# pyannote/pyannote-audio

Hardware: AMD Instinct MI355X
Metric: audio-hours/sec (real-time factor) for speaker-diarization-3.1 pipeline (higher is better)
Workload: dtype f32

## Files before the change

### pyannote-audio_amd/csrc/common.h

```cpp
#pragma once
#include <hip/hip_runtime.h>
#include <stdint.h>
#include <stdio.h>

typedef float f32x4 __attribute__((ext_vector_type(4)));
typedef float f32x16 __attribute__((ext_vector_type(16)));
typedef unsigned int u32x4 __attribute__((ext_vector_type(4)));

#define MFMA16(a, b, c) __builtin_amdgcn_mfma_f32_16x16x4f32((a), (b), (c), 0, 0, 0)
#define MFMA32(a, b, c) __builtin_amdgcn_mfma_f32_32x32x2f32((a), (b), (c), 0, 0, 0)

#define PA_INTERNAL __attribute__((visibility("hidden")))
PA_INTERNAL int pa_mfcc_frontend(const float* wav, long wav_len, long chunk_stride, int B, int N, int T, int hop,
                                 int center, int log_mels, const float* window, const float* fft_tw,
                                 const float* mel_w, const int* mel_lo, const int* mel_hi, int nmel,
                                 const float* dct, int n_mfcc, float* mel_buf, unsigned int* chunk_max, float* out,
                                 int rows, void* stream);
PA_INTERNAL int pa_stats_pool_rows_any(const float* feat, int B, int T0, int Tp, int C, int ld, const float* masks,
                                       int S, int Fm, const int* nearest_idx, float* stats, int ld_stats,
                                       const float* aff_scale, const float* aff_shift, void* stream);
PA_INTERNAL void pa_square_from_condensed(const double* cond, int n, long ld, double* S, void* stream);
PA_INTERNAL void pa_row_norms_f64(const double* X, int N, int D, double* nrm, void* stream);

#include "workspace.h"
namespace pa {

inline long square_ld(int n) { return ((long)n + 7) & ~7L; }
PA_INTERNAL bool square_fits(int n);

struct LfState {
  double *S, *mind0;
  int *nb0, *g_size, *g_cid;
  unsigned long long* mail;
  int* status;
};
PA_INTERNAL bool lf_wanted(int n);
PA_INTERNAL void lf_layout(Carver& c, int n, LfState& s);
PA_INTERNAL int lf_launch(const double* cond, int n, double* Z, const LfState& s, long long* stats, hipStream_t st);

void set_error(const char* fmt, ...);

hipError_t fill_async(void* dst, int value, size_t nbytes, hipStream_t st);

int* tile_counters();
}
#include "tile_queue.h"
namespace pa {

struct ProfScope {
  ProfScope(const char* name, void* stream, double flops, double bytes);
  ~ProfScope();
  long idx_;
  void* stream_;
};

#define PA_CHECK_LAUNCH(name)                                              \
  do {                                                                     \
    hipError_t e__ = hipGetLastError();                                    \
    if (e__ != hipSuccess) {                                               \
      pa::set_error("%s: launch failed: %s", name, hipGetErrorString(e__)); \
      return e__ == hipErrorOutOfMemory ? 2 : 1;                           \
    }                                                                      \
  } while (0)

#define PA_REQUIRE(cond, ...)        \
  do {                               \
    if (!(cond)) {                   \
      pa::set_error(__VA_ARGS__);    \
      return 3;                      \
    }                                \
  } while (0)

__device__ __forceinline__ float wave_sum(float v) {
#pragma unroll
  for (int o = 32; o > 0; o >>= 1) v += __shfl_xor(v, o, 64);
  return v;
}
__device__ __forceinline__ double wave_sum_d(double v) {
#pragma unroll
  for (int o = 32; o > 0; o >>= 1) v += __shfl_xor(v, o, 64);
  return v;
}

struct MinPair {
  double d;
  int i;
};
__device__ __forceinline__ MinPair min_pair(MinPair a, MinPair b) {
  if (b.i >= 0 && (a.i < 0 || b.d < a.d || (b.d == a.d && b.i < a.i))) return b;
  return a;
}

template <int NW>
__device__ __forceinline__ float block_sum(float v, float* red) {
  v = wave_sum(v);
  const int lane = threadIdx.x & 63, w = threadIdx.x >> 6;
  __syncthreads();
  if (lane == 0) red[w] = v;
  __syncthreads();
  float s = 0.f;
#pragma unroll
  for (int i = 0; i < NW; ++i) s += red[i];
  return s;
}

__device__ __forceinline__ float leaky_relu(float x) { return x > 0.f ? x : 0.01f * x; }
__device__ __forceinline__ float gelu_erf(float x) { return 0.5f * x * (1.f + erff(x * 0.70710678118654752440f)); }

static inline int cdiv(long a, long b) { return (int)((a + b - 1) / b); }

}
```

### pyannote-audio_amd/csrc/emb_fbank.hip

```cpp
#include "common.h"

namespace pa {

constexpr int FB_WIN = 400, FB_SHIFT = 160, FB_NFFT = 512, FB_HALF = 256, FB_NBIN = 257;
constexpr int FB_FPB = 4;

struct cplx {
  float x, y;
};
__device__ __forceinline__ cplx cmul(cplx a, cplx b) {
  return {a.x * b.x - a.y * b.y, a.x * b.y + a.y * b.x};
}

template <bool kRagged>
__global__ __launch_bounds__(256) void k_fbank(const float* __restrict__ wav, long wav_len,
                                               long chunk_stride, int T, float scale, float preemph,
                                               const float* __restrict__ window,
                                               const float2* __restrict__ tw256,
                                               const float2* __restrict__ tw512,
                                               const float* __restrict__ mel_w,
                                               const int* __restrict__ mel_lo,
                                               const int* __restrict__ mel_hi, int nmel, float eps,
                                               float* __restrict__ out, const int64_t* __restrict__ offs,
                                               const int* __restrict__ lens) {
  __shared__ float2 bufA[FB_FPB][FB_HALF];
  __shared__ float2 bufB[FB_FPB][FB_HALF];
  __shared__ float2 s_tw256[FB_HALF];
  __shared__ float xs[FB_FPB][FB_NFFT + 1];
  const int tid = threadIdx.x, lane = tid & 63, wv = tid >> 6;
  const int b = blockIdx.y;
  const int t = blockIdx.x * FB_FPB + wv;
  int Tb = T;
  long base = (long)b * chunk_stride + (long)t * FB_SHIFT;
  if constexpr (kRagged) {
    const int n = lens[b];
    Tb = n < FB_WIN ? 0 : 1 + (n - FB_WIN) / FB_SHIFT;
    if ((int)blockIdx.x * FB_FPB >= Tb) return;
    base = offs[b] + (long)t * FB_SHIFT;
  }
  for (int i = tid; i < FB_HALF; i += 256) s_tw256[i] = tw256[i];
  const bool active = t < Tb;
  float2 w512[5];
#pragma unroll
  for (int i = 0; i < 5; ++i) w512[i] = lane + 64 * i <= FB_HALF ? tw512[lane + 64 * i] : make_float2(0.f, 0.f);

  float x[7];
  float s = 0.f;
#pragma unroll
  for (int i = 0; i < 7; ++i) {
    const int j = lane + 64 * i;
    float v = 0.f;
    if (active && j < FB_WIN) {
      const long g = base + j;
      v = (g < wav_len ? wav[g] : 0.f) * scale;
    }
    x[i] = v;
    s += v;
  }
  const float mean = wave_sum(s) / (float)FB_WIN;
  float* xw = xs[wv];
#pragma unroll
  for (int i = 0; i < 7; ++i) {
    const int j = lane + 64 * i;
    if (j < FB_WIN) xw[j + 1] = x[i] - mean;
  }
  if (lane == 0) xw[0] = x[0] - mean;
  __syncthreads();
  float y[8];
#pragma unroll
  for (int i = 0; i < 8; ++i) {
    const int j = lane + 64 * i;
    float v = 0.f;
    if (j < FB_WIN) v = (xw[j + 1] - preemph * xw[j]) * window[j];
    y[i] = v;
  }
  __syncthreads();
#pragma unroll
  for (int i = 0; i < 8; ++i) xw[lane + 64 * i] = y[i];
  __syncthreads();
  float2* A = bufA[wv];
  float2* Bf = bufB[wv];
#pragma unroll
  for (int i = 0; i < 4; ++i) {
    const int n = lane + 64 * i;
    A[n] = make_float2(xw[2 * n], xw[2 * n + 1]);
  }
  __syncthreads();

  float2* src = A;
  float2* dst = Bf;
#pragma unroll
  for (int pass = 0; pass < 4; ++pass) {
    const int Ns = 1 << (2 * pass);
    const int j = lane;
    const int k = j & (Ns - 1);
    const int tstep = 64 >> (2 * pass);
    cplx v[4];
#pragma unroll
    for (int r = 0; r < 4; ++r) {
      const float2 d = src[j + 64 * r];
      const float2 w = s_tw256[(r * k * tstep) & 255];
      v[r] = cmul({d.x, d.y}, {w.x, w.y});
    }
    const cplx t0 = {v[0].x + v[2].x, v[0].y + v[2].y};
    const cplx t1 = {v[0].x - v[2].x, v[0].y - v[2].y};
    const cplx t2 = {v[1].x + v[3].x, v[1].y + v[3].y};
    const cplx d13 = {v[1].x - v[3].x, v[1].y - v[3].y};
    const cplx t3 = {d13.y, -d13.x};
    const int j0 = ((j - k) << 2) + k;
    dst[j0] = make_float2(t0.x + t2.x, t0.y + t2.y);
    dst[j0 + Ns] = make_float2(t1.x + t3.x, t1.y + t3.y);
    dst[j0 + 2 * Ns] = make_float2(t0.x - t2.x, t0.y - t2.y);
    dst[j0 + 3 * Ns] = make_float2(t1.x - t3.x, t1.y - t3.y);
    __syncthreads();
    float2* tmp = src;
    src = dst;
    dst = tmp;
  }
#pragma unroll
  for (int i = 0; i < 5; ++i) {
    const int k = lane + 64 * i;
    if (k <= FB_HALF) {
      const float2 zk = src[k & 255];
      const float2 zc0 = src[(FB_HALF - k) & 255];
      const cplx zc = {zc0.x, -zc0.y};
      const cplx e = {0.5f * (zk.x + zc.x), 0.5f * (zk.y + zc.y)};
      const cplx dd = {0.5f * (zk.x - zc.x), 0.5f * (zk.y - zc.y)};
      const cplx o = {dd.y, -dd.x};
      const float2 w = w512[i];
      const cplx wo = cmul(o, {w.x, w.y});
      const float re = e.x + wo.x, im = e.y + wo.y;
      xw[k] = re * re + im * im;
    }
  }
  __syncthreads();
  if (active) {
    for (int m = lane; m < nmel; m += 64) {
      const float* wrow = mel_w + (long)m * FB_NBIN;
      float acc = 0.f;
      const int lo = mel_lo[m], hi = mel_hi[m];
      for (int k0 = lo; k0 <= hi; k0 += 8) {
        float wk[8];
#pragma unroll
        for (int u = 0; u < 8; ++u) wk[u] = k0 + u <= hi ? wrow[k0 + u] : 0.f;
#pragma unroll
        for (int u = 0; u < 8; ++u)
          if (k0 + u <= hi) acc = fmaf(xw[k0 + u], wk[u], acc);
      }
      out[((long)b * T + t) * nmel + m] = logf(fmaxf(acc, eps));
    }
  }
}

__device__ __forceinline__ float fbank_frame_mean(const float* __restrict__ x, int T, int nmel, int m, int p,
                                                  double (*part)[80]) {
  double s = 0.0;
  if (m < nmel)
    for (int t = p; t < T; t += 4) s += (double)x[(long)t * nmel + m];
  part[p][m] = s;
  __syncthreads();
  return (float)((part[0][m] + part[1][m] + part[2][m] + part[3][m]) / (double)T);
}

__global__ __launch_bounds__(320) void k_fbank_center(float* __restrict__ fb, int T, int nmel) {
  __shared__ double part[4][80];
  const int b = blockIdx.x;
  const int m = threadIdx.x % 80, p = threadIdx.x / 80;
  float* x = fb + (long)b * T * nmel;
  const float mean = fbank_frame_mean(x, T, nmel, m, p, part);
  if (m < nmel)
    for (int t = p; t < T; t += 4) x[(long)t * nmel + m] -= mean;
}

__global__ __launch_bounds__(320) void k_fbank_center_ragged(float* __restrict__ fb, int T, int nmel,
                                                             const int* __restrict__ lens) {
  __shared__ double part[4][80];
  const int b = blockIdx.x;
  const int m = threadIdx.x % 80, p = threadIdx.x / 80;
  const int n = lens[b];
  const int Tb = n < FB_WIN ? 0 : 1 + (n - FB_WIN) / FB_SHIFT;
  float* x = fb + (long)b * T * nmel;
  const float mean = fbank_frame_mean(x, Tb, nmel, m, p, part);
  if (m < nmel) {
    for (int t = p; t < Tb; t += 4) x[(long)t * nmel + m] -= mean;
    for (int t = Tb + p; t < T; t += 4) x[(long)t * nmel + m] = 0.f;
  }
}

constexpr int FC_TT = 240, FC_MG = 16, FC_KMAX = 2049;
__global__ __launch_bounds__(256) void k_fbank_center_span(const float* __restrict__ fb, int T, int nmel, int K,
                                                           float* __restrict__ out) {
  extern __shared__ float fc_tile[];
  const int b = blockIdx.z, m0 = blockIdx.y * FC_MG, t0 = blockIdx.x * FC_TT;
  const int half = K >> 1;
  const int m = threadIdx.x & (FC_MG - 1), tl = threadIdx.x >> 4;
  const float* x = fb + (long)b * T * nmel;
  const int rows = FC_TT + K - 1;
  for (int r = tl; r < rows; r += 16) {
    const int t = t0 - half + r;
    fc_tile[r * FC_MG + m] = (t >= 0 && t < T && m0 + m < nmel) ? x[(long)t * nmel + m0 + m] : 0.f;
  }
  __syncthreads();
  if (m0 + m >= nmel) return;
  for (int i = tl; i < FC_TT; i += 16) {
    const int t = t0 + i;
    if (t >= T) break;
    const int lo = t - half < 0 ? 0 : t - half, hi = t + half > T - 1 ? T - 1 : t + half;
    float s = 0.f;
    for (int u = lo; u <= hi; ++u) s += fc_tile[(u - t0 + half) * FC_MG + m];
    out[((long)b * T + t) * nmel + m0 + m] = fc_tile[(i + half) * FC_MG + m] - s / (float)(hi - lo + 1);
  }
}

}

extern "C" {

int pa_fbank_center_span(const float* fb, int B, int T, int nmel, int kernel, float* out, void* stream) {
  PA_REQUIRE(kernel >= 1 && (kernel & 1), "pa_fbank_center_span: the window must be an odd number of frames (got %d)",
             kernel);
  PA_REQUIRE(fb != out, "pa_fbank_center_span: works out of place");
  if (B <= 0 || T <= 0 || nmel <= 0) return 0;
  if (kernel > 2 * T - 1) kernel = 2 * T - 1;
  PA_REQUIRE(kernel <= pa::FC_KMAX,
             "pa_fbank_center_span: a running mean over %d frames of a %d-frame chunk needs more than the LDS holds "
             "(at most %d frames)", kernel, T, pa::FC_KMAX);
  const size_t lds = (size_t)(pa::FC_TT + kernel - 1) * pa::FC_MG * sizeof(float);
  static bool attr_set = false;
  if (!attr_set) {
    (void)hipFuncSetAttribute((const void*)pa::k_fbank_center_span, hipFuncAttributeMaxDynamicSharedMemorySize,
                              (int)((pa::FC_TT + pa::FC_KMAX - 1) * pa::FC_MG * sizeof(float)));
    attr_set = true;
  }
  hipLaunchKernelGGL(pa::k_fbank_center_span, dim3(pa::cdiv(T, pa::FC_TT), pa::cdiv(nmel, pa::FC_MG), B), dim3(256), lds,
                     (hipStream_t)stream, fb, T, nmel, kernel, out);
  PA_CHECK_LAUNCH("pa_fbank_center_span");
  return 0;
}

int pa_fbank(const float* wav, long wav_len, long chunk_stride, int B, int N, const float* window,
             const float* tw256, const float* tw512, const float* mel_w, const int* mel_lo,
             const int* mel_hi, int nmel, float* out, int center, void* stream) {
  PA_REQUIRE(nmel <= 80, "pa_fbank: at most 80 mel bins are built (got %d)", nmel);
  if (B <= 0) return 0;
  PA_REQUIRE(N >= pa::FB_WIN, "pa_fbank: %d samples is shorter than one 25 ms frame", N);
  const int T = 1 + (N - pa::FB_WIN) / pa::FB_SHIFT;
  hipStream_t st = (hipStream_t)stream;
  pa::ProfScope prof("k_fbank", stream, (double)B * T * (5.0 * 512 * 9 + 2.0 * 257 * 3 + 2.0 * 257 * 2),
                     4.0 * B * N + 4.0 * B * T * nmel * (center ? 3 : 1));
  hipLaunchKernelGGL(pa::k_fbank<false>, dim3(pa::cdiv(T, pa::FB_FPB), B), dim3(256), 0, st, wav, wav_len,
                     chunk_stride, T, 32768.0f, 0.97f, window, (const float2*)tw256,
                     (const float2*)tw512, mel_w, mel_lo, mel_hi, nmel, 1.1920928955078125e-07f, out,
                     (const int64_t*)nullptr, (const int*)nullptr);
  PA_CHECK_LAUNCH("pa_fbank");
  if (center) {
    hipLaunchKernelGGL(pa::k_fbank_center, dim3(B), dim3(320), 0, st, out, T, nmel);
    PA_CHECK_LAUNCH("pa_fbank_center");
  }
  return 0;
}

int pa_fbank_ragged(const float* wav, long wav_len, const int64_t* offsets, const int32_t* lengths, int B,
                    int max_samples, const float* window, const float* tw256, const float* tw512, const float* mel_w,
                    const int* mel_lo, const int* mel_hi, int nmel, float* out, void* stream) {
  PA_REQUIRE(nmel <= 80, "pa_fbank_ragged: at most 80 mel bins are built (got %d)", nmel);
  if (B <= 0) return 0;
  PA_REQUIRE(max_samples >= pa::FB_WIN, "pa_fbank_ragged: %d samples is shorter than one 25 ms frame", max_samples);
  const int T = 1 + (max_samples - pa::FB_WIN) / pa::FB_SHIFT;
  hipStream_t st = (hipStream_t)stream;
  pa::ProfScope prof("k_fbank_ragged", stream, (double)B * T * (5.0 * 512 * 9 + 2.0 * 257 * 3 + 2.0 * 257 * 2),
                     4.0 * B * max_samples + 12.0 * B * T * nmel);
  hipLaunchKernelGGL(pa::k_fbank<true>, dim3(pa::cdiv(T, pa::FB_FPB), B), dim3(256), 0, st, wav, wav_len, 0L, T,
                     32768.0f, 0.97f, window, (const float2*)tw256, (const float2*)tw512, mel_w, mel_lo, mel_hi, nmel,
                     1.1920928955078125e-07f, out, offsets, (const int*)lengths);
  PA_CHECK_LAUNCH("pa_fbank_ragged");
  hipLaunchKernelGGL(pa::k_fbank_center_ragged, dim3(B), dim3(320), 0, st, out, T, nmel, (const int*)lengths);
  PA_CHECK_LAUNCH("pa_fbank_center_ragged");
  return 0;
}

}
```

### pyannote-audio_amd/csrc/emb_forward.cpp

```cpp
#include "forward_common.h"

namespace {

struct EmbPlan {
  int B, N, T, F, S;
  int Hs[5], Ws[5];
  size_t fbank, act[4], stats, total, act_elems;
  size_t t2_off, gather_off;
};

inline bool s2_fold_wanted() {
  static const bool fold = getenv("PA_S2_FOLD") == nullptr || atoi(getenv("PA_S2_FOLD")) != 0;
  return fold;
}

inline bool prefer_wino4(int H, int W, int cin) {
  auto up = [](int a, int b) { return (long)((a + b - 1) / b) * b; };
  long p4 = up(H, 4) * up(W, 64);
  const long p4_lin = up(H, 4) * up(W, 4);
  if (p4_lin * 120 <= p4 * 100) p4 = p4_lin * 120 / 100;
  long p2 = up(H, 8) * up(W, 32);
  if (up(H, 4) * up(W, 64) < p2) p2 = up(H, 4) * up(W, 64);
  if (up(H, 2) * up(W, 128) < p2) p2 = up(H, 2) * up(W, 128);
  const long gain = cin >= 256 ? 130 : 122;
  return p4 * 100 <= p2 * gain;
}

bool make_plan(const pa_emb_weights* w, int B, int N, int S, EmbPlan* p, bool calib = false) {
  if (N < 400) return false;
  p->B = B;
  p->N = N;
  p->S = S < 1 ? 1 : S;
  p->T = 1 + (N - 400) / 160;
  p->F = w->num_mel;
  p->Hs[0] = p->F;
  p->Ws[0] = p->T;
  for (int l = 0; l < w->num_layers; ++l) {
    const int s = l == 0 ? 1 : 2;
    p->Hs[l + 1] = (p->Hs[l] - 1) / s + 1;
    p->Ws[l + 1] = (p->Ws[l] - 1) / s + 1;
  }
  pa::Bump ws;
  p->fbank = ws.take((size_t)B * p->T * p->F);
  const int ex = w->bottleneck ? 4 : 1;
  p->act_elems = (size_t)B * p->Hs[0] * p->Ws[0] * w->planes[0] * ex;
  for (int i = 0; i < 3; ++i) p->act[i] = ws.take(p->act_elems);
  p->t2_off = p->gather_off = 0;
  if (w->bottleneck) {
    size_t t1 = 0, t2 = 0, g = 0;
    int cin = w->planes[0];
    for (int l = 0; l < w->num_layers; ++l) {
      const size_t planes = w->planes[l];
      const size_t in_px = (size_t)B * p->Hs[l == 0 ? 1 : l] * p->Ws[l == 0 ? 1 : l];
      const size_t out_px = (size_t)B * p->Hs[l + 1] * p->Ws[l + 1];
      t1 = t1 > in_px * planes ? t1 : in_px * planes;
      t2 = t2 > out_px * planes ? t2 : out_px * planes;
      if (l > 0) g = g > out_px * cin ? g : out_px * cin;
      cin = 4 * (int)planes;
    }
    p->t2_off = pa::Bump::align(t1);
    p->gather_off = p->t2_off + pa::Bump::align(t2);
    p->act[3] = ws.take(p->gather_off + pa::Bump::align(g));
  } else if (calib) {
    p->act[3] = ws.take(p->act_elems);
  }
  const int L = w->num_layers;
  p->stats = ws.take((size_t)B * p->S * 2 * w->planes[L - 1] * ex * p->Hs[L]);
  p->total = ws.o;
  return true;
}

}

extern "C" {

int pa_emb_num_fbank_frames(int num_samples) {
  return num_samples < 400 ? 0 : 1 + (num_samples - 400) / 160;
}

int pa_emb_num_pool_frames(const pa_emb_weights* w, int num_samples) {
  EmbPlan p;
  if (!make_plan(w, 1, num_samples, 1, &p)) return 0;
  return p.Ws[w->num_layers];
}

size_t pa_emb_workspace_bytes(const pa_emb_weights* w, int num_chunks, int num_samples, int num_masks) {
  EmbPlan p;
  if (!make_plan(w, num_chunks, num_samples, num_masks, &p)) return 0;
  return p.total * sizeof(float);
}

}


static int emb_forward_impl(const pa_emb_weights* w, const float* wav, int64_t wav_len, int64_t chunk_stride,
                            int num_chunks, int num_samples, const float* masks, int num_masks, int mask_frames,
                            const int32_t* nearest_idx, float* emb, void* workspace, size_t workspace_bytes,
                            void* stream, float* calib, const int64_t* offsets = nullptr,
                            const int32_t* lengths = nullptr) {
  if (num_chunks <= 0) return 0;
  const bool ragged = lengths != nullptr;
  EmbPlan p;
  if (w->num_layers != 4 || !make_plan(w, num_chunks, num_samples, masks ? num_masks : 1, &p, calib != nullptr)) {
    pa::set_error("pa_emb_forward: %d samples is too short (fbank needs >= 400) or bad layer count",
                  num_samples);
    return 3;
  }
  if (workspace_bytes < p.total * sizeof(float)) {
    pa::set_error("pa_emb_forward: workspace too small (%zu < %zu bytes)", workspace_bytes,
                  p.total * sizeof(float));
    return 3;
  }
  float* ws = (float*)workspace;
  const int B = p.B;

  const int span = w->fb_center_kernel;
  if (ragged && span != 0) {
    pa::set_error("pa_emb_forward_ragged: fbank_centering_span checkpoints run one launch sequence per length");
    return 3;
  }
  if (ragged)
    PA_RUN(pa_fbank_ragged(wav, wav_len, offsets, lengths, B, p.N, w->fb_window, w->fb_tw256, w->fb_tw512, w->fb_mel_w,
                           w->fb_mel_lo, w->fb_mel_hi, w->num_mel, ws + p.fbank, stream));
  else
    PA_RUN(pa_fbank(wav, wav_len, chunk_stride, B, p.N, w->fb_window, w->fb_tw256, w->fb_tw512, w->fb_mel_w,
                    w->fb_mel_lo, w->fb_mel_hi, w->num_mel, ws + p.fbank, span == 0 ? 1 : 0, stream));
  auto zero_tail = [&](float* X, int l, int C) -> int {
    return ragged ? pa_zero_tail_cols(X, B, p.Hs[l], p.Ws[l], C, lengths, l > 0 ? l - 1 : 0, stream) : 0;
  };
  float* cur = ws + p.act[0];
  float* f1 = ws + p.act[1];
  float* f2 = ws + p.act[2];
  const float* feats = ws + p.fbank;
  if (span != 0) {
    PA_RUN(pa_fbank_center_span(ws + p.fbank, B, p.T, p.F, span, f1, stream));
    feats = f1;
  }
  PA_RUN(pa_resnet_stem(feats, B, p.T, p.F, w->stem_w, w->stem_shift, cur, stream));
  if (!w->bottleneck) PA_RUN(zero_tail(cur, 0, w->planes[0]));

  auto conv_s1 = [&](const float* X, int H, int W, int ci, const float* v, const float* u, const float* wd,
                     const float* shift, const float* R, float* Y, int co, int slot) -> int {
    if (calib != nullptr) {
      float* scratch = ws + p.act[3];
      float* rep = calib + 4 * slot;
      const long n = (long)B * H * W * co;
      int r = pa_conv3x3(X, B, H, W, ci, wd, shift, R, Y, co, 1, 1, stream);
      if (r == 0 && v != nullptr) {
        r = pa_conv3x3_wino4(X, B, H, W, ci, v, shift, R, scratch, co, 1, stream);
        if (r == 0) r = pa_absmax_diff(scratch, Y, n, rep, stream);
      }
      if (r == 0 && u != nullptr) {
        r = pa_conv3x3_wino(X, B, H, W, ci, u, shift, R, scratch, co, 1, stream);
        if (r == 0) r = pa_absmax_diff(scratch, Y, n, rep + 2, stream);
      }
      return r;
    }
    if (v != nullptr && prefer_wino4(H, W, ci)) return pa_conv3x3_wino4(X, B, H, W, ci, v, shift, R, Y, co, 1, stream);
    if (u != nullptr) return pa_conv3x3_wino(X, B, H, W, ci, u, shift, R, Y, co, 1, stream);
    return pa_conv3x3(X, B, H, W, ci, wd, shift, R, Y, co, 1, 1, stream);
  };

  int blk = 0;
  int cin = w->planes[0];
  if (w->bottleneck) {
    float* nxt = f1;
    float* sc = f2;
    float* tmp = ws + p.act[3];
    for (int l = 0; l < w->num_layers; ++l) {
      const int planes = w->planes[l], cout = 4 * planes;
      for (int i = 0; i < w->num_blocks[l]; ++i, ++blk) {
        if (blk >= PA_MAX_RES_BLOCKS) {
          pa::set_error("pa_emb_forward: more than %d residual blocks", PA_MAX_RES_BLOCKS);
          return 3;
        }
        const int stride = (i == 0 && l > 0) ? 2 : 1;
        const int H = stride == 2 ? p.Hs[l] : p.Hs[l + 1], W = stride == 2 ? p.Ws[l] : p.Ws[l + 1];
        const int Ho = p.Hs[l + 1], Wo = p.Ws[l + 1];
        float* t1 = tmp;
        float* t2 = tmp + p.t2_off;
        PA_RUN(pa_gemm_tn_ex(cur, cin, w->blk_w1[blk], cin, w->blk_shift1[blk], nullptr, t1, planes, B * H * W,
                             planes, cin, 2, 0, stream));
        PA_RUN(zero_tail(t1, stride == 2 ? l : l + 1, planes));
        if (stride == 1 && w->blk_u2[blk] != nullptr)
          PA_RUN(pa_conv3x3_wino(t1, B, H, W, planes, w->blk_u2[blk], w->blk_shift2[blk], nullptr, t2, planes, 1,
                                 stream));
        else
          PA_RUN(pa_conv3x3(t1, B, H, W, planes, w->blk_w2[blk], w->blk_shift2[blk], nullptr, t2, planes, stride,
                            1, stream));
        const float* res = cur;
        if (w->blk_wsc[blk] != nullptr) {
          if (stride == 2)
            PA_RUN(pa_gemm_tn_s2(cur, B, H, W, cin, w->blk_wsc[blk], cin, w->blk_shiftsc[blk], sc, cout, cout, stream));
          else
            PA_RUN(pa_gemm_tn_ex(cur, cin, w->blk_wsc[blk], cin, w->blk_shiftsc[blk], nullptr, sc, cout,
                                 B * Ho * Wo, cout, cin, 0, 0, stream));
          res = sc;
        } else if (stride != 1 || cin != cout) {
          pa::set_error("pa_emb_forward: block %d needs a shortcut conv but none was given", blk);
          return 3;
        }
        PA_RUN(pa_gemm_tn_ex(t2, planes, w->blk_w3[blk], planes, w->blk_shift3[blk], res, nxt, cout, B * Ho * Wo,
                             cout, planes, 2, 0, stream));
        float* t = cur;
        cur = nxt;
        nxt = t;
        cin = cout;
      }
    }
  } else
  for (int l = 0; l < w->num_layers; ++l) {
    const int cout = w->planes[l];
    for (int i = 0; i < w->num_blocks[l]; ++i, ++blk) {
      if (blk >= PA_MAX_RES_BLOCKS) {
        pa::set_error("pa_emb_forward: more than %d residual blocks", PA_MAX_RES_BLOCKS);
        return 3;
      }
      const int stride = (i == 0 && l > 0) ? 2 : 1;
      const int H = stride == 2 ? p.Hs[l] : p.Hs[l + 1], W = stride == 2 ? p.Ws[l] : p.Ws[l + 1];
      const int Ho = p.Hs[l + 1], Wo = p.Ws[l + 1];
      if (w->blk_wsc[blk] != nullptr) {
        const size_t q = (size_t)B * Ho * Wo * cin;
        float* R = f2 + pa::Bump::align(q);
        const bool fold = stride == 2 && s2_fold_wanted() && pa_conv3x3_s2_sc_supported(H, cin, cout);
        if (fold)
          PA_RUN(pa_conv3x3_s2_sc(cur, B, H, W, cin, w->blk_w1[blk], w->blk_shift1[blk], w->blk_wsc[blk],
                                  w->blk_shiftsc[blk], f1, R, cout, 1, stream));
        else
          PA_RUN(pa_conv3x3(cur, B, H, W, cin, w->blk_w1[blk], w->blk_shift1[blk], nullptr, f1, cout, stride,
                            1, stream));
        PA_RUN(zero_tail(f1, l + 1, cout));
        if (fold) {
        } else if (stride == 2)
          PA_RUN(pa_gemm_tn_s2(cur, B, H, W, cin, w->blk_wsc[blk], cin, w->blk_shiftsc[blk], R, cout, cout, stream));
        else
          PA_RUN(pa_gemm_tn(cur, cin, w->blk_wsc[blk], cin, w->blk_shiftsc[blk], R, cout, B * Ho * Wo, cout, cin, 0, 0,
                            stream));
        PA_RUN(conv_s1(f1, Ho, Wo, cout, w->blk_v2[blk], w->blk_u2[blk], w->blk_w2[blk], w->blk_shift2[blk], R, cur,
                       cout, 2 * blk + 1));
        PA_RUN(zero_tail(cur, l + 1, cout));
      } else {
        if (stride != 1 || cin != cout) {
          pa::set_error("pa_emb_forward: block %d needs a shortcut conv but none was given", blk);
          return 3;
        }
        PA_RUN(conv_s1(cur, H, W, cin, w->blk_v1[blk], w->blk_u1[blk], w->blk_w1[blk], w->blk_shift1[blk], nullptr, f1,
                       cout, 2 * blk));
        PA_RUN(zero_tail(f1, l + 1, cout));
        PA_RUN(conv_s1(f1, H, W, cout, w->blk_v2[blk], w->blk_u2[blk], w->blk_w2[blk], w->blk_shift2[blk], cur, f2,
                       cout, 2 * blk + 1));
        PA_RUN(zero_tail(f2, l + 1, cout));
        float* t = cur;
        cur = f2;
        f2 = t;
      }
      cin = cout;
    }
  }
  const int L = w->num_layers;
  const int S = p.S;
  const int cfin = w->planes[L - 1] * (w->bottleneck ? 4 : 1);
  if (ragged)
    PA_RUN(pa_stats_pool_ragged(cur, B, p.Hs[L], p.Ws[L], cfin, lengths, L - 1, masks, p.Ws[L], ws + p.stats, stream));
  else
    PA_RUN(pa_stats_pool(cur, B, p.Hs[L], p.Ws[L], cfin, masks, S, mask_frames, nearest_idx, ws + p.stats, stream));
  const int D2 = 2 * cfin * p.Hs[L];
  PA_RUN(pa_gemm_tn(ws + p.stats, D2, w->seg1_w, D2, w->seg1_b, emb, w->embed_dim, B * S, w->embed_dim, D2,
                    0, 0, stream));
  return 0;
}

extern "C" {

int pa_emb_forward(const pa_emb_weights* w, const float* wav, int64_t wav_len, int64_t chunk_stride,
                   int num_chunks, int num_samples, const float* masks, int num_masks, int mask_frames,
                   const int32_t* nearest_idx, float* emb, void* workspace, size_t workspace_bytes,
                   void* stream) {
  return emb_forward_impl(w, wav, wav_len, chunk_stride, num_chunks, num_samples, masks, num_masks, mask_frames,
                          nearest_idx, emb, workspace, workspace_bytes, stream, nullptr);
}

size_t pa_emb_ragged_workspace_bytes(const pa_emb_weights* w, int num_utterances, int max_samples) {
  EmbPlan p;
  if (!make_plan(w, num_utterances, max_samples, 1, &p)) return 0;
  return p.total * sizeof(float);
}

int pa_emb_forward_ragged(const pa_emb_weights* w, const float* wav, int64_t wav_len, const int64_t* offsets,
                          const int32_t* lengths, int num_utterances, int max_samples, const float* masks, float* emb,
                          void* workspace, size_t workspace_bytes, void* stream) {
  if (offsets == nullptr || lengths == nullptr) {
    pa::set_error("pa_emb_forward_ragged: offsets and lengths are required");
    return 3;
  }
  return emb_forward_impl(w, wav, wav_len, 0, num_utterances, max_samples, masks, 1, 0, nullptr, emb, workspace,
                          workspace_bytes, stream, nullptr, offsets, lengths);
}

size_t pa_emb_calibrate_workspace_bytes(const pa_emb_weights* w, int num_chunks, int num_samples) {
  EmbPlan p;
  if (!make_plan(w, num_chunks, num_samples, 1, &p, true)) return 0;
  return p.total * sizeof(float);
}

int pa_emb_calibrate_winograd(const pa_emb_weights* w, const float* wav, int64_t wav_len, int64_t chunk_stride,
                              int num_chunks, int num_samples, float* report, float* emb, void* workspace,
                              size_t workspace_bytes, void* stream) {
  if (w->bottleneck) {
    pa::set_error("pa_emb_calibrate_winograd: BasicBlock networks only (Bottleneck blocks run F(2x2) / direct)");
    return 3;
  }
  if (pa::fill_async(report, 0, sizeof(float) * 8 * PA_MAX_RES_BLOCKS, (hipStream_t)stream) != hipSuccess) return 1;
  return emb_forward_impl(w, wav, wav_len, chunk_stride, num_chunks, num_samples, nullptr, 1, 0, nullptr, emb,
                          workspace, workspace_bytes, stream, report);
}

}
```

### pyannote-audio_amd/csrc/emb_resnet.hip

```cpp
#include "common.h"

namespace pa {

constexpr int STEM_TS = 64;
constexpr int STEM_LD = STEM_TS + 3;

__global__ __launch_bounds__(256) void k_stem(const float* __restrict__ fb, int T, int F,
                                              const float* __restrict__ w9,
                                              const float* __restrict__ shift,
                                              float* __restrict__ out) {
  extern __shared__ float xs[];
  const int b = blockIdx.y, t0 = blockIdx.x * STEM_TS;
  const int tid = threadIdx.x;
  for (int i = tid; i < 2 * STEM_LD; i += 256) xs[(i < STEM_LD ? 0 : (F + 1) * STEM_LD - STEM_LD) + i] = 0.f;
  const int n = (STEM_TS + 2) * F;
  for (int i0 = 0; i0 < n; i0 += 8 * 256) {
    float v[8];
#pragma unroll
    for (int k = 0; k < 8; ++k) {
      const int i = i0 + tid + 256 * k;
      const int tt = i / F, ff = i - tt * F, t = t0 + tt - 1;
      v[k] = (i < n && t >= 0 && t < T) ? fb[((long)b * T + t) * F + ff] : 0.f;
    }
#pragma unroll
    for (int k = 0; k < 8; ++k) {
      const int i = i0 + tid + 256 * k;
      const int tt = i / F, ff = i - tt * F;
      if (i < n) xs[(ff + 1) * STEM_LD + tt] = v[k];
    }
  }
  const int q4 = (tid & 7) * 4, pl = tid >> 3;
  float w[9][4], sh[4];
#pragma unroll
  for (int k = 0; k < 9; ++k)
#pragma unroll
    for (int c = 0; c < 4; ++c) w[k][c] = w9[k * 32 + q4 + c];
#pragma unroll
  for (int c = 0; c < 4; ++c) sh[c] = shift[q4 + c];
  __syncthreads();
  float x0[2][3], x1[2][3], x2[2][3];
#pragma unroll
  for (int h = 0; h < 2; ++h)
#pragma unroll
    for (int dt = 0; dt < 3; ++dt) {
      x0[h][dt] = xs[0 * STEM_LD + pl + 32 * h + dt];
      x1[h][dt] = xs[1 * STEM_LD + pl + 32 * h + dt];
    }
  const bool ok0 = t0 + pl < T, ok1 = t0 + pl + 32 < T;
  float* o = out + ((long)b * F * T + t0 + pl) * 32 + q4;
  for (int f = 0; f < F; ++f) {
#pragma unroll
    for (int h = 0; h < 2; ++h)
#pragma unroll
      for (int dt = 0; dt < 3; ++dt) x2[h][dt] = xs[(f + 2) * STEM_LD + pl + 32 * h + dt];
    float* of = o + (long)f * T * 32;
#pragma unroll
    for (int h = 0; h < 2; ++h) {
      float acc[4];
#pragma unroll
      for (int c = 0; c < 4; ++c) acc[c] = 0.f;
#pragma unroll
      for (int dt = 0; dt < 3; ++dt)
#pragma unroll
        for (int c = 0; c < 4; ++c) acc[c] = fmaf(x0[h][dt], w[dt][c], acc[c]);
#pragma unroll
      for (int dt = 0; dt < 3; ++dt)
#pragma unroll
        for (int c = 0; c < 4; ++c) acc[c] = fmaf(x1[h][dt], w[3 + dt][c], acc[c]);
#pragma unroll
      for (int dt = 0; dt < 3; ++dt)
#pragma unroll
        for (int c = 0; c < 4; ++c) acc[c] = fmaf(x2[h][dt], w[6 + dt][c], acc[c]);
      float4 o4;
      o4.x = fmaxf(acc[0] + sh[0], 0.f);
      o4.y = fmaxf(acc[1] + sh[1], 0.f);
      o4.z = fmaxf(acc[2] + sh[2], 0.f);
      o4.w = fmaxf(acc[3] + sh[3], 0.f);
      if (h == 0 ? ok0 : ok1) *reinterpret_cast<float4*>(of + 32 * 32 * h) = o4;
    }
#pragma unroll
    for (int h = 0; h < 2; ++h)
#pragma unroll
      for (int dt = 0; dt < 3; ++dt) {
        x0[h][dt] = x1[h][dt];
        x1[h][dt] = x2[h][dt];
      }
  }
}

constexpr int CB = 16;
constexpr int CLD = CB + 4;

template <int TH, int TWT>
struct ConvGeom {
  static constexpr int TW = 32 * TWT;
  static constexpr int PH = TH + 2;
  static constexpr int PW = TW + 2;
  static constexpr int PATCH = PH * PW * CLD;
};

template <int TH, int TWT, int BN, bool HAS_R>
__global__ __launch_bounds__(256, 2) void k_conv3x3(const float* __restrict__ X, int H, int W, int CIN,
                                                    const float* __restrict__ Wg,
                                                    const float* __restrict__ shift,
                                                    const float* __restrict__ R, float* __restrict__ Y,
                                                    int Ho, int Wo, int COUT, int relu, int tiles_w,
                                                    int tiles_hw, int n_tiles, int total_tiles, int xranges,
                                                    int* __restrict__ counters) {
  using G = ConvGeom<TH, TWT>;
  constexpr int MT = TH * TWT;
  constexpr int MPW = MT / 4;
  constexpr int NT = BN / 32;
  static_assert(MT % 4 == 0, "M-tiles must split over 4 waves");
  extern __shared__ __attribute__((aligned(16))) float smem[];
  float* patch = smem;
  float* wts = smem + G::PATCH;

  const int tid = threadIdx.x, lane = tid & 63, wv = tid >> 6;
  const int li = lane & 31, kh = lane >> 5;
  constexpr int NPF4 = G::PH * G::PW * (CB / 4);
  constexpr int NP = (NPF4 + 255) / 256;
  constexpr int NWF4 = 9 * BN * (CB / 4);
  constexpr int NW = (NWF4 + 255) / 256;
  constexpr int OOB = (int)0x80000000;

  struct Tile {
    int b, n0, y0, x0;
  };
  const int num_pb = total_tiles / n_tiles;
  auto pair_of = [&](int t) {
    return xranges ? (t & 7) * ((num_pb + 7) >> 3) + (t >> 3) / n_tiles : ((t >> 3) / n_tiles) * 8 + (t & 7);
  };
  auto decode = [&](int t) {
    Tile q;
    const int pb = pair_of(t);
    q.n0 = (((t >> 3) % n_tiles)) * BN;
    const int pix = pb % tiles_hw;
    q.b = pb / tiles_hw;
    q.y0 = (pix / tiles_w) * TH;
    q.x0 = (pix % tiles_w) * G::TW;
    return q;
  };
  auto resolve = [&](const TileQueue& tqq, int r) {
    for (;;) {
      const int t = tq_resolve(tqq, r);
      if (t < 0 || pair_of(t) < num_pb) return t;
      r = tq_claim_own(tqq);
    }
  };
  u32x4 rp[NP], rw[NW];
  struct Offs {
    int p[NP];
  };
  int offw[NW];
#pragma unroll
  for (int e = 0; e < NW; ++e) {
    const int i = tid + 256 * e;
    const int c4 = i & 3, rn = i >> 2;
    const int tap = rn / BN, n = rn % BN;
    offw[e] = (NWF4 % 256 == 0 || i < NWF4) ? ((tap * COUT + n) * CIN + 4 * c4) * 4 : OOB;
  }
  auto tile_offsets = [&](const Tile& q, Offs& o) {
#pragma unroll
    for (int e = 0; e < NP; ++e) {
      const int i = tid + 256 * e;
      const int c4 = i & 3, pp = i >> 2;
      const int py = pp / G::PW, px = pp % G::PW;
      const int iy = q.y0 - 1 + py, ix = q.x0 - 1 + px;
      o.p[e] = ((NPF4 % 256 == 0 || i < NPF4) && iy >= 0 && iy < H && ix >= 0 && ix < W)
                   ? ((iy * W + ix) * CIN + 4 * c4) * 4
                   : OOB;
    }
  };
  auto gload = [&](const Tile& q, int c0) {
    const __amdgpu_buffer_rsrc_t xsrd = __builtin_amdgcn_make_buffer_rsrc(
        const_cast<float*>(X + (long)q.b * H * W * CIN), 0, H * W * CIN * 4, 0x00020000);
    const __amdgpu_buffer_rsrc_t wsrd = __builtin_amdgcn_make_buffer_rsrc(
        const_cast<float*>(Wg + (long)q.n0 * CIN), 0, (9 * COUT - q.n0) * CIN * 4, 0x00020000);
    Offs here;
    tile_offsets(q, here);
#pragma unroll
    for (int e = 0; e < NP; ++e) rp[e] = __builtin_amdgcn_raw_buffer_load_b128(xsrd, here.p[e], c0 * 4, 0);
#pragma unroll
    for (int e = 0; e < NW; ++e) rw[e] = __builtin_amdgcn_raw_buffer_load_b128(wsrd, offw[e], c0 * 4, 0);
  };
  auto lstore = [&]() {
#pragma unroll
    for (int e = 0; e < NP; ++e) {
      const int i = tid + 256 * e;
      const int c4 = i & 3, pp = i >> 2;
      if (NPF4 % 256 == 0 || i < NPF4) *reinterpret_cast<u32x4*>(patch + pp * CLD + 4 * c4) = rp[e];
    }
#pragma unroll
    for (int e = 0; e < NW; ++e) {
      const int i = tid + 256 * e;
      if (NWF4 % 256 == 0 || i < NWF4)
        *reinterpret_cast<u32x4*>(wts + (i >> 2) * CLD + 4 * (i & 3)) = rw[e];
    }
  };

  __shared__ int s_next;
  const TileQueue tq{counters, (int)(blockIdx.x & 7), ((num_pb + 7) >> 3) * n_tiles};
  if (tid == 0) s_next = resolve(tq, tq_claim_own(tq));
  __syncthreads();
  int t = s_next;
  if (t < 0) {
    if (tid == 0) tq_done(tq, gridDim.x);
    return;
  }
  Tile cur = decode(t);
  gload(cur, 0);
  for (;;) {
    int ahead = 0;
    if (tid == 0) ahead = tq_claim_own(tq);
    int tn = -1;
    f32x16 acc[MPW][NT];
#pragma unroll
    for (int i = 0; i < MPW; ++i)
#pragma unroll
      for (int j = 0; j < NT; ++j)
#pragma unroll
        for (int r = 0; r < 16; ++r) acc[i][j][r] = 0.f;
    Tile nxt = cur;

    for (int c0 = 0; c0 < CIN; c0 += CB) {
      __syncthreads();
      lstore();
      if (c0 == 0 && tid == 0) s_next = resolve(tq, ahead);
      __syncthreads();
      if (c0 == 0) {
        tn = s_next;
        if (tn >= 0) nxt = decode(tn);
      }
      if (c0 + CB < CIN) gload(cur, c0 + CB);
      else if (tn >= 0) gload(nxt, 0);
      float4 af[1][MPW][2], bf[1][NT][2];
      auto load_tap = [&](int tap, float4 (&a)[MPW][2], float4 (&bq)[NT][2]) {
        const int dy = tap / 3, dx = tap % 3;
#pragma unroll
        for (int i = 0; i < MPW; ++i) {
          const int mt = wv * MPW + i;
          const int yy = mt / TWT, xt = mt % TWT;
          const int off = ((yy + dy) * G::PW + 32 * xt + li + dx) * CLD;
          a[i][0] = *reinterpret_cast<const float4*>(patch + off + kh * 8);
          a[i][1] = *reinterpret_cast<const float4*>(patch + off + kh * 8 + 4);
        }
#pragma unroll
        for (int j = 0; j < NT; ++j) {
          const int off = (tap * BN + 32 * j + li) * CLD + kh * 8;
          bq[j][0] = *reinterpret_cast<const float4*>(wts + off);
          bq[j][1] = *reinterpret_cast<const float4*>(wts + off + 4);
        }
      };
      auto mfma_tap = [&](const float4 (&a)[MPW][2], const float4 (&bq)[NT][2]) {
#pragma unroll
        for (int h = 0; h < 2; ++h)
#pragma unroll
          for (int i = 0; i < MPW; ++i)
#pragma unroll
            for (int j = 0; j < NT; ++j) {
              acc[i][j] = MFMA32(a[i][h].x, bq[j][h].x, acc[i][j]);
              acc[i][j] = MFMA32(a[i][h].y, bq[j][h].y, acc[i][j]);
              acc[i][j] = MFMA32(a[i][h].z, bq[j][h].z, acc[i][j]);
              acc[i][j] = MFMA32(a[i][h].w, bq[j][h].w, acc[i][j]);
            }
      };
#pragma unroll 1
      for (int dy = 0; dy < 3; ++dy)
#pragma unroll
        for (int dx = 0; dx < 3; ++dx) {
          load_tap(dy * 3 + dx, af[0], bf[0]);
          mfma_tap(af[0], bf[0]);
        }
    }
    {
      const __amdgpu_buffer_rsrc_t ysrd = __builtin_amdgcn_make_buffer_rsrc(
          Y + (long)cur.b * Ho * Wo * COUT, 0, Ho * Wo * COUT * 4, 0x00020000);
      const __amdgpu_buffer_rsrc_t rsrd = __builtin_amdgcn_make_buffer_rsrc(
          const_cast<float*>(HAS_R ? R + (long)cur.b * Ho * Wo * COUT : Y), 0,
          Ho * Wo * COUT * 4, 0x00020000);
      constexpr int NG = MPW * NT;
      int off[2][16];
      float rv[2][16];
      auto goffs = [&](int g, int* o) {
        const int i = g / NT, j = g % NT;
        const int mt = wv * MPW + i;
        const int y = cur.y0 + mt / TWT, xbase = cur.x0 + 32 * (mt % TWT) + 4 * kh;
        const int n = cur.n0 + 32 * j + li;
#pragma unroll
        for (int r = 0; r < 16; ++r) {
          const int x = xbase + (r & 3) + 8 * (r >> 2);
          o[r] = (y < Ho && x < Wo) ? ((y * Wo + x) * COUT + n) * 4 : OOB;
        }
      };
      auto gres = [&](const int* o, float* v) {
        if (HAS_R) {
#pragma unroll
          for (int r = 0; r < 16; ++r)
            v[r] = __builtin_bit_cast(float, __builtin_amdgcn_raw_buffer_load_b32(rsrd, o[r], 0, 0));
        } else {
#pragma unroll
          for (int r = 0; r < 16; ++r) v[r] = 0.f;
        }
      };
      goffs(0, off[0]);
      gres(off[0], rv[0]);
#pragma unroll
      for (int g = 0; g < NG; ++g) {
        if (g + 1 < NG) {
          goffs(g + 1, off[(g + 1) & 1]);
          gres(off[(g + 1) & 1], rv[(g + 1) & 1]);
        }
        const int i = g / NT, j = g % NT;
        const float sh = shift[cur.n0 + 32 * j + li];
#pragma unroll
        for (int r = 0; r < 16; ++r) {
          float v = acc[i][j][r] + sh + rv[g & 1][r];
          if (relu) v = fmaxf(v, 0.f);
          __builtin_amdgcn_raw_buffer_store_b32(__builtin_bit_cast(unsigned int, v), ysrd, off[g & 1][r], 0, 0);
        }
      }
    }
    if (tn < 0) break;
    cur = nxt;
  }
  if (tid == 0) tq_done(tq, gridDim.x);
}

int xcd_ranges_wanted(bool by_default);
int launch_conv_s2(const float* X, int B, int H, int W, int CIN, const float* Wg, const float* shift, const float* R,
                   float* Y, int COUT, int relu, hipStream_t st);
int launch_conv_s2_sc(const float* X, int B, int H, int W, int CIN, const float* Wg, const float* shift,
                      const float* Wsc, const float* shift_sc, float* Y, float* Ysc, int COUT, int relu,
                      hipStream_t st);

template <int TH, int TWT, int BN, bool HAS_R>
static int launch_conv_r(const float* X, int B, int H, int W, int CIN, const float* Wg,
                         const float* shift, const float* R, float* Y, int COUT, int relu,
                         hipStream_t st) {
  using G = ConvGeom<TH, TWT>;
  const int Ho = H, Wo = W;
  const int tiles_w = cdiv(Wo, G::TW), tiles_h = cdiv(Ho, TH);
  const size_t lds = (size_t)(G::PATCH + 9 * BN * CLD) * sizeof(float);
  constexpr int MAXDEV = 16;
  static int resident_of[MAXDEV] = {0}, per_cu_of[MAXDEV] = {0};
  int dev = 0;
  (void)hipGetDevice(&dev);
  if (dev < 0 || dev >= MAXDEV) dev = 0;
  if (!resident_of[dev]) {
    (void)hipFuncSetAttribute((const void*)k_conv3x3<TH, TWT, BN, HAS_R>,
                              hipFuncAttributeMaxDynamicSharedMemorySize, (int)lds);
    int cus = 256, per_cu = 2;
    (void)hipDeviceGetAttribute(&cus, hipDeviceAttributeMultiprocessorCount, dev);
    if (hipOccupancyMaxActiveBlocksPerMultiprocessor(&per_cu, k_conv3x3<TH, TWT, BN, HAS_R>, 256, lds) !=
            hipSuccess || per_cu < 1)
      per_cu = 2;
    resident_of[dev] = cus * per_cu;
    per_cu_of[dev] = per_cu;
  }
  const int resident = resident_of[dev] & ~7;
  const int tiles_hw = tiles_w * tiles_h, n_tiles = COUT / BN;
  const long total = (long)tiles_hw * n_tiles * B;
  const int grid = (int)(total < resident ? total : resident);
  int* counters = tile_counters();
  if (counters == nullptr) {
    set_error("pa_conv3x3: cannot allocate the tile counters");
    return 2;
  }
  hipLaunchKernelGGL((k_conv3x3<TH, TWT, BN, HAS_R>), dim3(grid), dim3(256), lds, st, X, H, W, CIN, Wg,
                     shift, R, Y, Ho, Wo, COUT, relu, tiles_w, tiles_hw, n_tiles, (int)total, xcd_ranges_wanted(true),
                     counters);
  return 0;
}

template <int TH, int TWT, int BN>
static int launch_conv(const float* X, int B, int H, int W, int CIN, const float* Wg,
                       const float* shift, const float* R, float* Y, int COUT, int relu,
                       hipStream_t st) {
  return R != nullptr ? launch_conv_r<TH, TWT, BN, true>(X, B, H, W, CIN, Wg, shift, R, Y, COUT, relu, st)
                      : launch_conv_r<TH, TWT, BN, false>(X, B, H, W, CIN, Wg, shift, R, Y, COUT, relu, st);
}

}

extern "C" {

int pa_resnet_stem(const float* fbank, int B, int T, int F, const float* w9, const float* shift,
                   float* out, void* stream) {
  if (B <= 0) return 0;
  pa::ProfScope prof("k_stem", stream, 2.0 * B * T * F * 9 * 32, 4.0 * B * T * F * 33);
  PA_REQUIRE(F >= 1 && (size_t)(F + 2) * pa::STEM_LD * 4 <= 64 * 1024, "pa_resnet_stem: %d mel bins do not fit LDS", F);
  hipLaunchKernelGGL(pa::k_stem, dim3(pa::cdiv(T, pa::STEM_TS), B), dim3(256), (size_t)(F + 2) * pa::STEM_LD * 4,
                     (hipStream_t)stream, fbank, T, F, w9, shift, out);
  PA_CHECK_LAUNCH("pa_resnet_stem");
  return 0;
}

int pa_conv3x3(const float* X, int B, int H, int W, int cin, const float* Wg, const float* shift,
               const float* R, float* Y, int cout, int stride, int relu, void* stream) {
  if (B <= 0) return 0;
  PA_REQUIRE(cin % pa::CB == 0 && cout % 32 == 0, "pa_conv3x3: cin %% 16 and cout %% 32 required");
  hipStream_t st = (hipStream_t)stream;
  const int Ho = (H - 1) / stride + 1, Wo_ = (W - 1) / stride + 1;
  pa::ProfScope prof("k_conv3x3", stream, 2.0 * 9 * cin * cout * (double)B * Ho * Wo_,
                     4.0 * ((double)B * H * W * cin + (double)B * Ho * Wo_ * cout * (R ? 2 : 1) + 9.0 * cin * cout));
  if (stride == 1) {
    int rc;
    if (cout == 32) rc = pa::launch_conv<8, 1, 32>(X, B, H, W, cin, Wg, shift, R, Y, cout, relu, st);
    else if (Ho >= 32) rc = pa::launch_conv<8, 1, 64>(X, B, H, W, cin, Wg, shift, R, Y, cout, relu, st);
    else if (Ho >= 16) rc = pa::launch_conv<4, 2, 64>(X, B, H, W, cin, Wg, shift, R, Y, cout, relu, st);
    else rc = pa::launch_conv<2, 2, 64>(X, B, H, W, cin, Wg, shift, R, Y, cout, relu, st);
    if (rc != 0) return rc;
  } else if (stride == 2) {
    PA_REQUIRE(cout % 64 == 0, "pa_conv3x3: stride 2 needs cout %% 64 == 0");
    if (pa::launch_conv_s2(X, B, H, W, cin, Wg, shift, R, Y, cout, relu, st) != 0) return 2;
  } else {
    PA_REQUIRE(false, "pa_conv3x3: stride %d not supported", stride);
  }
  PA_CHECK_LAUNCH("pa_conv3x3");
  return 0;
}

int pa_conv3x3_s2_sc_supported(int H, int cin, int cout) {
  return H >= 1 && cin >= pa::CB && cin % pa::CB == 0 && cout >= 64 && cout % 64 == 0 && (H - 1) / 2 + 1 >= 16;
}

int pa_conv3x3_s2_sc(const float* X, int B, int H, int W, int cin, const float* Wg, const float* shift,
                     const float* Wsc, const float* shift_sc, float* Y, float* Ysc, int cout, int relu,
                     void* stream) {
  if (B <= 0) return 0;
  PA_REQUIRE(cin >= pa::CB && cin % pa::CB == 0, "pa_conv3x3_s2_sc: cin %% 16 == 0 required");
  PA_REQUIRE(cout >= 64 && cout % 64 == 0, "pa_conv3x3_s2_sc: cout %% 64 == 0 required");
  const int Ho = (H - 1) / 2 + 1, Wo_ = (W - 1) / 2 + 1;
  PA_REQUIRE(H >= 1 && W >= 1 && Ho >= 16, "pa_conv3x3_s2_sc: at least 16 output rows required (got %d)", Ho);
  const size_t n_out = (size_t)B * Ho * Wo_ * cout;
  PA_REQUIRE(Y != nullptr && Ysc != nullptr && (Y + n_out <= Ysc || Ysc + n_out <= Y),
             "pa_conv3x3_s2_sc: Y and Ysc overlap");
  pa::ProfScope prof("k_conv3x3", stream, 2.0 * (9 + 1) * cin * cout * (double)B * Ho * Wo_,
                     4.0 * ((double)B * H * W * cin + 2.0 * (double)B * Ho * Wo_ * cout + 10.0 * cin * cout));
  if (pa::launch_conv_s2_sc(X, B, H, W, cin, Wg, shift, Wsc, shift_sc, Y, Ysc, cout, relu, (hipStream_t)stream) != 0)
    return 2;
  PA_CHECK_LAUNCH("pa_conv3x3_s2_sc");
  return 0;
}

}
```

Before: 1.333.

## Share fbank frames across overlapping embedding chunks and fold centering into stem

```diff
diff --git a/pyannote-audio_amd/csrc/common.h b/pyannote-audio_amd/csrc/common.h
--- a/pyannote-audio_amd/csrc/common.h
+++ b/pyannote-audio_amd/csrc/common.h
@@ -19,6 +19,11 @@
 PA_INTERNAL int pa_stats_pool_rows_any(const float* feat, int B, int T0, int Tp, int C, int ld, const float* masks,
                                        int S, int Fm, const int* nearest_idx, float* stats, int ld_stats,
                                        const float* aff_scale, const float* aff_shift, void* stream);
+PA_INTERNAL int pa_fbank_shared(const float* wav, long wav_len, int fps, int B, int N, const float* window,
+                                const float* tw256, const float* tw512, const float* mel_w, const int* mel_lo,
+                                const int* mel_hi, int nmel, float* frames, float* mean, void* stream);
+PA_INTERNAL int pa_resnet_stem_frames(const float* frames, int fps, const float* mean, int B, int T, int F,
+                                      const float* w9, const float* shift, float* out, void* stream);
 PA_INTERNAL void pa_square_from_condensed(const double* cond, int n, long ld, double* S, void* stream);
 PA_INTERNAL void pa_row_norms_f64(const double* X, int N, int D, double* nrm, void* stream);
 
diff --git a/pyannote-audio_amd/csrc/emb_fbank.hip b/pyannote-audio_amd/csrc/emb_fbank.hip
--- a/pyannote-audio_amd/csrc/emb_fbank.hip
+++ b/pyannote-audio_amd/csrc/emb_fbank.hip
@@ -172,6 +172,15 @@
     for (int t = p; t < T; t += 4) x[(long)t * nmel + m] -= mean;
 }
 
+__global__ __launch_bounds__(320) void k_fbank_chunk_mean(const float* __restrict__ frames, int fps, int T, int nmel,
+                                                          float* __restrict__ mean) {
+  __shared__ double part[4][80];
+  const int b = blockIdx.x;
+  const int m = threadIdx.x % 80, p = threadIdx.x / 80;
+  const float v = fbank_frame_mean(frames + (long)b * fps * nmel, T, nmel, m, p, part);
+  if (m < nmel) mean[(long)b * nmel + m] = v;
+}
+
 __global__ __launch_bounds__(320) void k_fbank_center_ragged(float* __restrict__ fb, int T, int nmel,
                                                              const int* __restrict__ lens) {
   __shared__ double part[4][80];
@@ -212,6 +221,30 @@
   }
 }
 
+}
+
+int pa_fbank_shared(const float* wav, long wav_len, int fps, int B, int N, const float* window, const float* tw256,
+                    const float* tw512, const float* mel_w, const int* mel_lo, const int* mel_hi, int nmel,
+                    float* frames, float* mean, void* stream) {
+  PA_REQUIRE(nmel <= 80, "pa_fbank_shared: at most 80 mel bins are built (got %d)", nmel);
+  if (B <= 0) return 0;
+  PA_REQUIRE(N >= pa::FB_WIN && fps >= 1, "pa_fbank_shared: %d samples every %d frames", N, fps);
+  const int T = 1 + (N - pa::FB_WIN) / pa::FB_SHIFT;
+  const long Ff = (long)(B - 1) * fps + T;
+  PA_REQUIRE(Ff <= 0x7fffffffL, "pa_fbank_shared: %ld frames in one launch", Ff);
+  hipStream_t st = (hipStream_t)stream;
+  {
+    pa::ProfScope prof("k_fbank", stream, (double)Ff * (5.0 * 512 * 9 + 2.0 * 257 * 3 + 2.0 * 257 * 2),
+                       4.0 * ((double)(Ff - 1) * pa::FB_SHIFT + pa::FB_WIN) + 4.0 * Ff * nmel);
+    hipLaunchKernelGGL(pa::k_fbank<false>, dim3(pa::cdiv(Ff, pa::FB_FPB), 1), dim3(256), 0, st, wav, wav_len, 0L,
+                       (int)Ff, 32768.0f, 0.97f, window, (const float2*)tw256, (const float2*)tw512, mel_w, mel_lo,
+                       mel_hi, nmel, 1.1920928955078125e-07f, frames, (const int64_t*)nullptr, (const int*)nullptr);
+    PA_CHECK_LAUNCH("pa_fbank_shared");
+  }
+  pa::ProfScope prof("k_fbank_chunk_mean", stream, (double)B * T * nmel, 4.0 * B * T * nmel + 4.0 * B * nmel);
+  hipLaunchKernelGGL(pa::k_fbank_chunk_mean, dim3(B), dim3(320), 0, st, (const float*)frames, fps, T, nmel, mean);
+  PA_CHECK_LAUNCH("pa_fbank_chunk_mean");
+  return 0;
 }
 
 extern "C" {
diff --git a/pyannote-audio_amd/csrc/emb_forward.cpp b/pyannote-audio_amd/csrc/emb_forward.cpp
--- a/pyannote-audio_amd/csrc/emb_forward.cpp
+++ b/pyannote-audio_amd/csrc/emb_forward.cpp
@@ -12,6 +12,11 @@
 inline bool s2_fold_wanted() {
   static const bool fold = getenv("PA_S2_FOLD") == nullptr || atoi(getenv("PA_S2_FOLD")) != 0;
   return fold;
+}
+
+inline bool shared_fbank_wanted() {
+  const char* e = getenv("PA_EMB_SHARED_FBANK");
+  return e == nullptr || atoi(e) != 0;
 }
 
 inline bool prefer_wino4(int H, int W, int cin) {
@@ -119,7 +124,16 @@
     pa::set_error("pa_emb_forward_ragged: fbank_centering_span checkpoints run one launch sequence per length");
     return 3;
   }
-  if (ragged)
+  const int64_t fps = chunk_stride > 0 && chunk_stride % 160 == 0 ? chunk_stride / 160 : 0;
+  const size_t span_frames = (size_t)(B - 1) * (size_t)fps + p.T;
+  const bool shared = !ragged && span == 0 && fps > 0 && B >= 2 && shared_fbank_wanted() &&
+                      fps < p.T  &&
+                      (span_frames + B) * p.F <= (size_t)B * p.T * p.F;
+  if (shared)
+    PA_RUN(pa_fbank_shared(wav, wav_len, (int)fps, B, p.N, w->fb_window, w->fb_tw256, w->fb_tw512, w->fb_mel_w,
+                           w->fb_mel_lo, w->fb_mel_hi, w->num_mel, ws + p.fbank, ws + p.fbank + span_frames * p.F,
+                           stream));
+  else if (ragged)
     PA_RUN(pa_fbank_ragged(wav, wav_len, offsets, lengths, B, p.N, w->fb_window, w->fb_tw256, w->fb_tw512, w->fb_mel_w,
                            w->fb_mel_lo, w->fb_mel_hi, w->num_mel, ws + p.fbank, stream));
   else
@@ -136,7 +150,11 @@
     PA_RUN(pa_fbank_center_span(ws + p.fbank, B, p.T, p.F, span, f1, stream));
     feats = f1;
   }
-  PA_RUN(pa_resnet_stem(feats, B, p.T, p.F, w->stem_w, w->stem_shift, cur, stream));
+  if (shared)
+    PA_RUN(pa_resnet_stem_frames(feats, (int)fps, feats + span_frames * p.F, B, p.T, p.F, w->stem_w, w->stem_shift, cur,
+                                 stream));
+  else
+    PA_RUN(pa_resnet_stem(feats, B, p.T, p.F, w->stem_w, w->stem_shift, cur, stream));
   if (!w->bottleneck) PA_RUN(zero_tail(cur, 0, w->planes[0]));
 
   auto conv_s1 = [&](const float* X, int H, int W, int ci, const float* v, const float* u, const float* wd,
diff --git a/pyannote-audio_amd/csrc/emb_resnet.hip b/pyannote-audio_amd/csrc/emb_resnet.hip
--- a/pyannote-audio_amd/csrc/emb_resnet.hip
+++ b/pyannote-audio_amd/csrc/emb_resnet.hip
@@ -5,7 +5,9 @@
 constexpr int STEM_TS = 64;
 constexpr int STEM_LD = STEM_TS + 3;
 
-__global__ __launch_bounds__(256) void k_stem(const float* __restrict__ fb, int T, int F,
+template <bool kCentred>
+__global__ __launch_bounds__(256) void k_stem(const float* __restrict__ fb, int fps, const float* __restrict__ mean,
+                                              int T, int F,
                                               const float* __restrict__ w9,
                                               const float* __restrict__ shift,
                                               float* __restrict__ out) {
@@ -16,16 +18,20 @@
   const int n = (STEM_TS + 2) * F;
   for (int i0 = 0; i0 < n; i0 += 8 * 256) {
     float v[8];
+    [[maybe_unused]] float mu[8];
 #pragma unroll
     for (int k = 0; k < 8; ++k) {
       const int i = i0 + tid + 256 * k;
       const int tt = i / F, ff = i - tt * F, t = t0 + tt - 1;
-      v[k] = (i < n && t >= 0 && t < T) ? fb[((long)b * T + t) * F + ff] : 0.f;
+      const bool in = i < n && t >= 0 && t < T;
+      v[k] = in ? fb[((long)b * fps + t) * F + ff] : 0.f;
+      if constexpr (kCentred) mu[k] = in ? mean[(long)b * F + ff] : 0.f;
     }
 #pragma unroll
     for (int k = 0; k < 8; ++k) {
       const int i = i0 + tid + 256 * k;
       const int tt = i / F, ff = i - tt * F;
+      if constexpr (kCentred) v[k] -= mu[k];
       if (i < n) xs[(ff + 1) * STEM_LD + tt] = v[k];
     }
   }
@@ -383,17 +389,29 @@
 
 }
 
+int pa_resnet_stem_frames(const float* frames, int fps, const float* mean, int B, int T, int F, const float* w9,
+                          const float* shift, float* out, void* stream) {
+  if (B <= 0) return 0;
+  const double read = mean != nullptr ? ((double)(B - 1) * fps + T + B) * F : (double)B * T * F;
+  pa::ProfScope prof("k_stem", stream, 2.0 * B * T * F * 9 * 32, 4.0 * (read + 32.0 * B * T * F));
+  PA_REQUIRE(F >= 1 && (size_t)(F + 2) * pa::STEM_LD * 4 <= 64 * 1024, "pa_resnet_stem: %d mel bins do not fit LDS", F);
+  const dim3 grid(pa::cdiv(T, pa::STEM_TS), B);
+  const size_t lds = (size_t)(F + 2) * pa::STEM_LD * 4;
+  if (mean != nullptr)
+    hipLaunchKernelGGL(pa::k_stem<true>, grid, dim3(256), lds, (hipStream_t)stream, frames, fps, mean, T, F, w9, shift,
+                       out);
+  else
+    hipLaunchKernelGGL(pa::k_stem<false>, grid, dim3(256), lds, (hipStream_t)stream, frames, fps, mean, T, F, w9, shift,
+                       out);
+  PA_CHECK_LAUNCH("pa_resnet_stem");
+  return 0;
+}
+
 extern "C" {
 
 int pa_resnet_stem(const float* fbank, int B, int T, int F, const float* w9, const float* shift,
                    float* out, void* stream) {
-  if (B <= 0) return 0;
-  pa::ProfScope prof("k_stem", stream, 2.0 * B * T * F * 9 * 32, 4.0 * B * T * F * 33);
-  PA_REQUIRE(F >= 1 && (size_t)(F + 2) * pa::STEM_LD * 4 <= 64 * 1024, "pa_resnet_stem: %d mel bins do not fit LDS", F);
-  hipLaunchKernelGGL(pa::k_stem, dim3(pa::cdiv(T, pa::STEM_TS), B), dim3(256), (size_t)(F + 2) * pa::STEM_LD * 4,
-                     (hipStream_t)stream, fbank, T, F, w9, shift, out);
-  PA_CHECK_LAUNCH("pa_resnet_stem");
-  return 0;
+  return pa_resnet_stem_frames(fbank, T, nullptr, B, T, F, w9, shift, out, stream);
 }
 
 int pa_conv3x3(const float* X, int B, int H, int W, int cin, const float* Wg, const float* shift,
```

Measured after the change: 1.348, median of 6. 1.01x the previous value.
